# jonregef/sihl

Measured on NVIDIA B200. Metric: det-head images/sec (assign+loss+NMS), higher is better.
Workload: dtype f32

## Files before the change

### sihl_b200/csrc/od_nms.cu

```cuda
#include "od_common.cuh"

namespace sihl {

constexpr int kNmsThreads = 1024;
constexpr int kSmemItems = 4096;
constexpr int kBigSegment = 512;
constexpr int kSmallItems = 256;
static_assert(4 * kSmallItems == kNmsThreads, "short-list path: four lanes per candidate");
constexpr size_t kSmemItemBytes = 47;
constexpr size_t kWsItemBytes = 48;

__device__ __forceinline__ unsigned f2ord_nms(float f)
{
    const unsigned u = __float_as_uint(f);
    return (u & 0x80000000u) ? ~u : (u | 0x80000000u);
}

struct NmsArrays {
    unsigned long long *key;
    float4 *box;
    unsigned *val;
    float *area;
    unsigned *slot;
    int *seg;
    unsigned char *dead;
};

__device__ __forceinline__ NmsArrays carve(unsigned char *base, int np)
{
    NmsArrays a;
    a.key = reinterpret_cast<unsigned long long *>(base);
    a.box = reinterpret_cast<float4 *>(base + (size_t)np * 8);
    a.val = reinterpret_cast<unsigned *>(base + (size_t)np * 24);
    a.area = reinterpret_cast<float *>(base + (size_t)np * 28);
    a.slot = reinterpret_cast<unsigned *>(base + (size_t)np * 32);
    a.seg = reinterpret_cast<int *>(base + (size_t)np * 36);
    a.dead = base + (size_t)np * 40;
    return a;
}

template <bool DESC>
__device__ __forceinline__ void bitonic_kv(unsigned long long *key, unsigned *val, int np)
{
    for (int k = 2; k <= np; k <<= 1)
        for (int j = k >> 1; j > 0; j >>= 1) {
            for (int i = threadIdx.x; i < np; i += blockDim.x) {
                const int ixj = i ^ j;
                if (ixj > i) {
                    const unsigned long long a = key[i], b = key[ixj];
                    const bool first = (i & k) == 0;
                    const bool swap = DESC ? (first ? (a < b) : (a > b)) : (first ? (a > b) : (a < b));
                    if (swap) {
                        key[i] = b; key[ixj] = a;
                        if (val) { const unsigned t = val[i]; val[i] = val[ixj]; val[ixj] = t; }
                    }
                }
            }
            __syncthreads();
        }
}

template <class Flag, class Emit>
__device__ __forceinline__ int block_ordered_compact(int n, int *s_warp , Flag flag, Emit emit)
{
    const int lane = threadIdx.x & 31, warp = threadIdx.x >> 5, nwarps = blockDim.x >> 5;
    int running = 0;
    for (int i0 = 0; i0 < n; i0 += blockDim.x) {
        const int i = i0 + threadIdx.x;
        const bool f = i < n && flag(i);
        const unsigned m = __ballot_sync(kFullMask, f);
        if (lane == 0) s_warp[warp] = __popc(m);
        __syncthreads();
        if (warp == 0) {
            const int x = lane < nwarps ? s_warp[lane] : 0;
            int incl = x;
#pragma unroll
            for (int o = 1; o < 32; o <<= 1) {
                const int y = __shfl_up_sync(kFullMask, incl, o);
                if (lane >= o) incl += y;
            }
            if (lane < nwarps) s_warp[lane] = incl - x;
            if (lane == 31) s_warp[32] = incl;
        }
        __syncthreads();
        if (f) emit(i, running + s_warp[warp] + __popc(m & ((1u << lane) - 1u)));
        running += s_warp[32];
        __syncthreads();
    }
    return running;
}

__device__ __forceinline__ bool iou_gt(float4 a, float area_a, float4 b, float area_b, float thr)
{
    const float w = fmaxf(0.f, fminf(a.z, b.z) - fmaxf(a.x, b.x));
    const float h = fmaxf(0.f, fminf(a.w, b.w) - fmaxf(a.y, b.y));
    const float inter = w * h;
    return inter / ((area_a + area_b) - inter) > thr;
}

__device__ __forceinline__ float4 shfl4(float4 v, int src)
{
    return make_float4(__shfl_sync(kFullMask, v.x, src), __shfl_sync(kFullMask, v.y, src), __shfl_sync(kFullMask, v.z, src),
                       __shfl_sync(kFullMask, v.w, src));
}

__device__ __forceinline__ unsigned chunk_greedy(float4 bi, float ai, bool dead, float thr, int lane)
{
    unsigned over = 0u;
#pragma unroll 4
    for (int l = 0; l < 31; ++l) {
        const float4 bl = shfl4(bi, l);
        const float al = __shfl_sync(kFullMask, ai, l);
        if (l < lane && iou_gt(bl, al, bi, ai, thr)) over |= 1u << l;
    }
    const unsigned alive = __ballot_sync(kFullMask, !dead);
    unsigned kept = 0u;
#pragma unroll 4
    for (int l = 0; l < 32; ++l) {
        const unsigned ol = __shfl_sync(kFullMask, over, l);
        if (((alive >> l) & 1u) && (ol & kept) == 0u) kept |= 1u << l;
    }
    return kept;
}

template <bool SMEM>
__device__ __forceinline__ void warp_segment_nms(const float4 *box, const float *area, unsigned char *dead_flag, int q0, int m,
                                                 float thr, int lane)
{
    if (SMEM) { __builtin_assume(__isShared(box)); __builtin_assume(__isShared(area)); __builtin_assume(__isShared(dead_flag)); }
    else { __builtin_assume(__isGlobal(box)); __builtin_assume(__isGlobal(area)); __builtin_assume(__isGlobal(dead_flag)); }
    for (int c0 = 0; c0 < m; c0 += 32) {
        __syncwarp();
        const int i = c0 + lane;
        const bool valid = i < m;
        const float4 bi = valid ? box[q0 + i] : make_float4(0.f, 0.f, 0.f, 0.f);
        const float ai = valid ? area[q0 + i] : 0.f;
        const bool dead = valid ? dead_flag[q0 + i] != 0 : true;
        const unsigned kept = chunk_greedy(bi, ai, dead, thr, lane);
        if (valid && !dead && !((kept >> lane) & 1u)) dead_flag[q0 + i] = 1;
        for (int j0 = c0 + 32; j0 < m; j0 += 32) {
            const int j = j0 + lane;
            const bool live = j < m && dead_flag[q0 + j] == 0;
            const float4 bj = live ? box[q0 + j] : make_float4(0.f, 0.f, 0.f, 0.f);
            const float aj = live ? area[q0 + j] : 0.f;
            bool kill = false;
            for (unsigned k = kept; k != 0u; k &= k - 1u) {
                const int l = __ffs(k) - 1;
                const float4 bl = shfl4(bi, l);
                const float al = __shfl_sync(kFullMask, ai, l);
                if (live && !kill && iou_gt(bl, al, bj, aj, thr)) kill = true;
            }
            if (kill) dead_flag[q0 + j] = 1;
        }
    }
}

struct ChunkScratch { float4 box[32]; float area[32]; unsigned kept; int n_big; int big[32]; };

template <bool SMEM>
__device__ __forceinline__ void cta_segment_nms(const float4 *box, const float *area, unsigned char *dead_flag, int q0, int m,
                                                float thr, ChunkScratch *sc)
{
    if (SMEM) { __builtin_assume(__isShared(box)); __builtin_assume(__isShared(area)); __builtin_assume(__isShared(dead_flag)); }
    else { __builtin_assume(__isGlobal(box)); __builtin_assume(__isGlobal(area)); __builtin_assume(__isGlobal(dead_flag)); }
    __builtin_assume(__isShared(sc));
    const int tid = threadIdx.x, lane = tid & 31, warp = tid >> 5;
    for (int c0 = 0; c0 < m; c0 += 32) {
        __syncthreads();
        if (warp == 0) {
            const int i = c0 + lane;
            const bool valid = i < m;
            const float4 bi = valid ? box[q0 + i] : make_float4(0.f, 0.f, 0.f, 0.f);
            const float ai = valid ? area[q0 + i] : 0.f;
            const bool dead = valid ? dead_flag[q0 + i] != 0 : true;
            const unsigned kept = chunk_greedy(bi, ai, dead, thr, lane);
            if (valid && !dead && !((kept >> lane) & 1u)) dead_flag[q0 + i] = 1;
            sc->box[lane] = bi;
            sc->area[lane] = ai;
            if (lane == 0) sc->kept = kept;
        }
        __syncthreads();
        const unsigned kept = sc->kept;
        if (kept == 0u) continue;
        for (int j = c0 + 32 + tid; j < m; j += blockDim.x) {
            if (dead_flag[q0 + j]) continue;
            const float4 bj = box[q0 + j];
            const float aj = area[q0 + j];
            for (unsigned k = kept; k != 0u; k &= k - 1u) {
                const int l = __ffs(k) - 1;
                if (iou_gt(sc->box[l], sc->area[l], bj, aj, thr)) { dead_flag[q0 + j] = 1; break; }
            }
        }
    }
    __syncthreads();
}

struct NmsParams {
    const int32_t *cand_count; int64_t cap;
    const unsigned long long *cand_key; const float4 *cand_box; const int32_t *cand_cls;
    const float4 *boxes; const float *scores; const int64_t *classes; const int32_t *seg_offsets;
    int mode;
    float iou_thr;
    int K; int64_t *num_instances; float *out_scores; int64_t *out_classes; float4 *out_boxes;
    int64_t *keep; int32_t *keep_count;
    unsigned char *workspace; size_t ws_stride;
    int reset_counts;
    const int32_t *list_offsets;
    unsigned long long *out_keys;
    int smem_items;
};

__device__ __forceinline__ int64_t list_base(const NmsParams &p, int img)
{
    return p.list_offsets != nullptr ? (int64_t)__ldg(p.list_offsets + img) : (int64_t)img * p.cap;
}
__device__ __forceinline__ unsigned char *list_workspace(const NmsParams &p, int img, int src0)
{
    if (p.mode != 0) return p.workspace + (size_t)2 * src0 * kWsItemBytes;
    if (p.list_offsets != nullptr) return p.workspace + (size_t)2 * __ldg(p.list_offsets + img) * kWsItemBytes;
    return p.workspace + (size_t)img * p.ws_stride;
}

__device__ __forceinline__ void nms_big_body(const NmsParams &p)
{
    extern __shared__ __align__(16) unsigned char s_dyn[];
    __shared__ int s_warp[33];

    const int img = blockIdx.x, tid = threadIdx.x, lane = tid & 31, warp = tid >> 5, nwarps = blockDim.x >> 5;
    const int64_t lb = p.mode == 0 ? list_base(p, img) : 0;
    int n, src0;
    if (p.mode == 0) {
        const int c = __ldg(p.cand_count + img);
        n = (int)(c < p.cap ? c : p.cap);
        src0 = 0;
    } else {
        src0 = __ldg(p.seg_offsets + img);
        n = __ldg(p.seg_offsets + img + 1) - src0;
    }
    int np = 2;
    while (np < n) np <<= 1;
    int n_kept = 0;

    if (n > 0) {
        unsigned char *base = s_dyn;
        if (np > p.smem_items)
            base = list_workspace(p, img, src0);
        const NmsArrays ar = carve(base, np);

        for (int i = tid; i < np; i += blockDim.x) {
            unsigned long long key = 0ull;
            if (i < n) {
                if (p.mode == 0) key = __ldg(p.cand_key + lb + i);
                else key = ((unsigned long long)f2ord_nms(__ldg(p.scores + src0 + i)) << 32) |
                           (unsigned long long)(0xffffffffu - (unsigned)i);
            }
            ar.key[i] = key;
            ar.val[i] = (unsigned)i;
        }
        __syncthreads();
        bitonic_kv<true>(ar.key, ar.val, np);

        for (int r = tid; r < np; r += blockDim.x) {
            unsigned long long key = ~0ull;
            if (r < n) {
                const unsigned slot = ar.val[r];
                const unsigned c = p.mode == 0 ? (unsigned)__ldg(p.cand_cls + lb + slot)
                                               : (unsigned)__ldg(p.classes + src0 + slot);
                key = ((unsigned long long)c << 32) | (unsigned long long)r;
            }
            ar.key[r] = key;
        }
        __syncthreads();
        bitonic_kv<false>(ar.key, nullptr, np);
        for (int q = tid; q < n; q += blockDim.x) {
            const unsigned r = (unsigned)(ar.key[q] & 0xffffffffu), slot = ar.val[r];
            const float4 bx = p.mode == 0 ? __ldg(p.cand_box + lb + slot) : __ldg(p.boxes + src0 + slot);
            ar.box[q] = bx;
            ar.area[q] = (bx.z - bx.x) * (bx.w - bx.y);
            ar.slot[q] = slot;
            ar.dead[q] = 0;
        }
        __syncthreads();
        for (int q = tid; q < n; q += blockDim.x) ar.val[(unsigned)(ar.key[q] & 0xffffffffu)] = (unsigned)q;

        const int n_seg = block_ordered_compact(
            n, s_warp, [&](int q) { return q == 0 || (ar.key[q] >> 32) != (ar.key[q - 1] >> 32); },
            [&](int q, int s) { ar.seg[s] = q; });
        if (tid == 0) ar.seg[n_seg] = n;
        __syncthreads();
        bool any_big = false;
        for (int s = warp; s < n_seg; s += nwarps) {
            const int q0 = ar.seg[s], m = ar.seg[s + 1] - q0;
            if (m > kBigSegment) continue;
            for (int i = 0; i + 1 < m; ++i) {
                __syncwarp();
                if (ar.dead[q0 + i]) continue;
                const float4 bi = ar.box[q0 + i];
                const float ai = ar.area[q0 + i];
                for (int j = i + 1 + lane; j < m; j += 32)
                    if (!ar.dead[q0 + j] && iou_gt(bi, ai, ar.box[q0 + j], ar.area[q0 + j], p.iou_thr)) ar.dead[q0 + j] = 1;
            }
        }
        for (int s = 0; s < n_seg; ++s) any_big |= (ar.seg[s + 1] - ar.seg[s]) > kBigSegment;
        __syncthreads();
        if (any_big) {
            for (int s = 0; s < n_seg; ++s) {
                const int q0 = ar.seg[s], m = ar.seg[s + 1] - q0;
                if (m <= kBigSegment) continue;
                for (int i = 0; i + 1 < m; ++i) {
                    __syncthreads();
                    if (ar.dead[q0 + i]) continue;
                    const float4 bi = ar.box[q0 + i];
                    const float ai = ar.area[q0 + i];
                    for (int j = i + 1 + tid; j < m; j += blockDim.x)
                        if (!ar.dead[q0 + j] && iou_gt(bi, ai, ar.box[q0 + j], ar.area[q0 + j], p.iou_thr))
                            ar.dead[q0 + j] = 1;
                }
                __syncthreads();
            }
        }

        n_kept = block_ordered_compact(
            n, s_warp, [&](int r) { return ar.dead[ar.val[r]] == 0; },
            [&](int r, int k) {
                const unsigned q = ar.val[r], slot = ar.slot[q];
                if (p.mode == 0) {
                    if (k < p.K) {
                        const int64_t o = (int64_t)img * p.K + k;
                        const unsigned long long ck = __ldg(p.cand_key + lb + slot);
                        p.out_scores[o] = __uint_as_float((unsigned)(ck >> 32));
                        p.out_classes[o] = (int64_t)(ar.key[q] >> 32);
                        p.out_boxes[o] = ar.box[q];
                        if (p.out_keys != nullptr) p.out_keys[o] = ck;
                    }
                } else {
                    p.keep[src0 + k] = (int64_t)src0 + slot;
                }
            });
    }

    if (p.mode == 0) {
        const int m = n_kept < p.K ? n_kept : p.K;
        if (tid == 0) {
            p.num_instances[img] = m;
            if (p.reset_counts) const_cast<int32_t *>(p.cand_count)[img] = 0;
        }
        for (int k = m + tid; k < p.K; k += blockDim.x) {
            const int64_t o = (int64_t)img * p.K + k;
            p.out_scores[o] = 0.f;
            p.out_classes[o] = 0;
            p.out_boxes[o] = make_float4(0.f, 0.f, 0.f, 0.f);
        }
    } else if (tid == 0) {
        p.keep_count[img] = n_kept;
    }
}

__device__ __forceinline__ int nms_small_body(const NmsParams &p, const int *sel = nullptr, int n_sel = 0, bool finalize = true)
{
    __shared__ unsigned long long s_key[kSmallItems];
    __shared__ unsigned s_cls[kSmallItems];
    __shared__ float4 s_box[kSmallItems];
    __shared__ float s_area[kSmallItems];
    __shared__ unsigned s_mask[kSmallItems];
    __shared__ unsigned s_keep[kSmallItems];
    __shared__ unsigned char s_dead[kSmallItems];
    __shared__ unsigned short s_q_of_r[kSmallItems], s_slot_of_r[kSmallItems], s_seg0_of_q[kSmallItems], s_len_of_q[kSmallItems];
    __shared__ int s_warp[33];
    __shared__ int s_big;

    const int img = blockIdx.x, tid = threadIdx.x, lane = tid & 31;
    const int64_t lb = p.mode == 0 ? list_base(p, img) : 0;
    const int item = tid >> 2, sub = tid & 3;
    int n, src0;
    if (p.mode == 0) {
        const int c = __ldg(p.cand_count + img);
        n = (int)(c < p.cap ? c : p.cap);
        src0 = 0;
    } else {
        src0 = __ldg(p.seg_offsets + img);
        n = __ldg(p.seg_offsets + img + 1) - src0;
    }
    if (sel != nullptr) n = n_sel;
    int n_kept = 0;
    if (n > 0) {
        const bool have = item < n;
        unsigned long long key = 0ull;
        unsigned cls = 0;
        float4 bx = make_float4(0.f, 0.f, 0.f, 0.f);
        if (have) {
            if (p.mode == 0) {
                const int src = sel != nullptr ? sel[item] : item;
                key = __ldg(p.cand_key + lb + src);
                cls = (unsigned)__ldg(p.cand_cls + lb + src);
                bx = __ldg(p.cand_box + lb + src);
            } else {
                key = ((unsigned long long)f2ord_nms(__ldg(p.scores + src0 + item)) << 32) |
                      (unsigned long long)(0xffffffffu - (unsigned)item);
                cls = (unsigned)__ldg(p.classes + src0 + item);
                bx = __ldg(p.boxes + src0 + item);
            }
            if (sub == 0) { s_key[item] = key; s_cls[item] = cls; }
        }
        if (tid == 0) s_big = 0;
        if (sub == 0 && item < kSmallItems) {
            s_q_of_r[item] = 0; s_slot_of_r[item] = 0; s_seg0_of_q[item] = 0; s_len_of_q[item] = 1; s_mask[item] = 0u;
            s_keep[item] = 0u; s_dead[item] = 0; s_box[item] = make_float4(0.f, 0.f, 0.f, 0.f); s_area[item] = 0.f;
        }
        __syncthreads();
        int r = 0, seg0 = 0, k = 0, len = 0;
        if (have) {
#pragma unroll 4
            for (int j = sub; j < n; j += 4) {
                const unsigned long long kj = s_key[j];
                const unsigned cj = s_cls[j];
                const bool better = kj > key, same = cj == cls;
                r += better;
                seg0 += cj < cls;
                k += same && better;
                len += same;
            }
        }
#pragma unroll
        for (int o = 2; o > 0; o >>= 1) {
            r += __shfl_xor_sync(kFullMask, r, o);
            seg0 += __shfl_xor_sync(kFullMask, seg0, o);
            k += __shfl_xor_sync(kFullMask, k, o);
            len += __shfl_xor_sync(kFullMask, len, o);
        }
        const int q = seg0 + k;
        if (have && sub == 0) {
            s_box[q] = bx;
            s_area[q] = (bx.z - bx.x) * (bx.w - bx.y);
            s_q_of_r[r] = (unsigned short)q;
            s_slot_of_r[r] = (unsigned short)item;
            s_seg0_of_q[q] = (unsigned short)seg0;
            s_len_of_q[q] = (unsigned short)len;
            s_dead[q] = 0;
            if (len > 32) s_big = 1;
        }
        __syncthreads();
        unsigned mask = 0;
        if (have && len <= 32) {
            const float area = (bx.z - bx.x) * (bx.w - bx.y);
            for (int j = sub; j < k; j += 4)
                if (iou_gt(s_box[seg0 + j], s_area[seg0 + j], bx, area, p.iou_thr)) mask |= 1u << j;
        }
        mask |= __shfl_xor_sync(kFullMask, mask, 1);
        mask |= __shfl_xor_sync(kFullMask, mask, 2);
        if (have && sub == 0) s_mask[q] = mask;
        __syncthreads();
        if (have && sub == 0 && k == 0 && len <= 32) {
            unsigned kept = 1u;
            for (int i = 1; i < len; ++i)
                if ((s_mask[seg0 + i] & kept) == 0u) kept |= 1u << i;
            s_keep[seg0] = kept;
        }
        __syncthreads();
        if (s_big) {
            const int warp = tid >> 5, nwarps = blockDim.x >> 5;
            for (int qq = warp; qq < n; qq += nwarps) {
                const int q0 = s_seg0_of_q[qq], m = s_len_of_q[qq];
                if (qq != q0 || m <= 32) continue;
                for (int i = 0; i + 1 < m; ++i) {
                    __syncwarp();
                    if (s_dead[q0 + i]) continue;
                    const float4 bi = s_box[q0 + i];
                    const float ai = s_area[q0 + i];
                    for (int j = i + 1 + lane; j < m; j += 32)
                        if (!s_dead[q0 + j] && iou_gt(bi, ai, s_box[q0 + j], s_area[q0 + j], p.iou_thr)) s_dead[q0 + j] = 1;
                }
            }
            __syncthreads();
        }
        n_kept = block_ordered_compact(
            n, s_warp,
            [&](int rr) {
                const int qq = s_q_of_r[rr], q0 = s_seg0_of_q[qq];
                return s_len_of_q[qq] <= 32 ? ((s_keep[q0] >> (qq - q0)) & 1u) != 0u : s_dead[qq] == 0;
            },
            [&](int rr, int kk) {
                const int qq = s_q_of_r[rr], slot = s_slot_of_r[rr];
                if (p.mode == 0) {
                    if (kk < p.K) {
                        const int64_t o = (int64_t)img * p.K + kk;
                        p.out_scores[o] = __uint_as_float((unsigned)(s_key[slot] >> 32));
                        p.out_classes[o] = (int64_t)s_cls[slot];
                        p.out_boxes[o] = s_box[qq];
                        if (p.out_keys != nullptr) p.out_keys[o] = s_key[slot];
                    }
                } else {
                    p.keep[src0 + kk] = (int64_t)src0 + slot;
                }
            });
    }
    if (!finalize) return n_kept;
    if (p.mode == 0) {
        const int m = n_kept < p.K ? n_kept : p.K;
        if (tid == 0) {
            p.num_instances[img] = m;
            if (p.reset_counts) const_cast<int32_t *>(p.cand_count)[img] = 0;
        }
        for (int kk = m + tid; kk < p.K; kk += blockDim.x) {
            const int64_t o = (int64_t)img * p.K + kk;
            p.out_scores[o] = 0.f;
            p.out_classes[o] = 0;
            p.out_boxes[o] = make_float4(0.f, 0.f, 0.f, 0.f);
        }
    } else if (tid == 0) {
        p.keep_count[img] = n_kept;
    }
    return n_kept;
}

constexpr int kLazyTarget = 200;
constexpr int kLazyMaxK = 128;
__device__ __forceinline__ int lazy_prefix_select(const NmsParams &p, int64_t lb, int n, int *s_sel, unsigned *s_hist,
                                                  unsigned *s_pick, int *s_count)
{
    const int tid = threadIdx.x, lane = tid & 31;
    unsigned prefix = 0u, mask = 0u, remaining = (unsigned)kLazyTarget;
    for (int pass = 0; pass < 4; ++pass) {
        const int shift = 24 - 8 * pass;
        for (int i = tid; i < 256; i += blockDim.x) s_hist[i] = 0u;
        __syncthreads();
        for (int i0 = 0; i0 < n; i0 += blockDim.x) {
            const int i = i0 + tid;
            const bool ok = i < n;
            const unsigned u = ok ? (unsigned)(__ldg(p.cand_key + lb + i) >> 32) : 0u;
            const bool in = ok && ((u & mask) == prefix);
            const unsigned digit = (u >> shift) & 255u;
            const unsigned act = __ballot_sync(kFullMask, in);
            if (in) {
                const unsigned peers = __match_any_sync(act, digit);
                if (lane == __ffs(peers) - 1) atomicAdd(&s_hist[digit], (unsigned)__popc(peers));
            }
        }
        __syncthreads();
        if (tid < 32) {
            unsigned c[8], tot = 0u;
#pragma unroll
            for (int j = 0; j < 8; ++j) { c[j] = s_hist[255 - (lane * 8 + j)]; tot += c[j]; }
            unsigned incl = tot;
#pragma unroll
            for (int o = 1; o < 32; o <<= 1) {
                const unsigned y = __shfl_up_sync(kFullMask, incl, o);
                if (lane >= o) incl += y;
            }
            unsigned before = incl - tot;
            if (before < remaining && remaining <= incl) {
#pragma unroll
                for (int j = 0; j < 8; ++j) {
                    if (before < remaining && remaining <= before + c[j]) {
                        s_pick[0] = 255u - (unsigned)(lane * 8 + j);
                        s_pick[1] = remaining - before;
                    }
                    before += c[j];
                }
            }
        }
        __syncthreads();
        prefix |= s_pick[0] << shift;
        mask |= 255u << shift;
        remaining = s_pick[1];
        __syncthreads();
    }
    if (tid == 0) *s_count = 0;
    __syncthreads();
    for (int i0 = 0; i0 < n; i0 += blockDim.x) {
        const int i = i0 + tid;
        if (i < n && (unsigned)(__ldg(p.cand_key + lb + i) >> 32) >= prefix) {
            const int pos = atomicAdd(s_count, 1);
            if (pos < kSmallItems) s_sel[pos] = i;
        }
    }
    __syncthreads();
    const int c = *s_count;
    return c <= kSmallItems ? c : 0;
}

constexpr int kWarpSegment = 2048;
constexpr int kHashSlots = 1024;
constexpr unsigned kHashEmpty = 0xffffffffu;
constexpr size_t kMedItemBytes = 47;
static_assert(kMedItemBytes <= kSmemItemBytes && kMedItemBytes <= kWsItemBytes, "long-list layouts must fit the shared/workspace strides");

struct MedArrays {
    unsigned long long *u_key;
    unsigned long long *f_key;
    float4 *f_box;
    unsigned *u_slot, *f_slot;
    float *f_area;
    unsigned short *b_id;
    unsigned char *f_dead;
};

__device__ __forceinline__ MedArrays carve_med(unsigned char *base, int n_al)
{
    MedArrays a;
    a.u_key = reinterpret_cast<unsigned long long *>(base);
    a.f_key = reinterpret_cast<unsigned long long *>(base + (size_t)n_al * 8);
    a.f_box = reinterpret_cast<float4 *>(base + (size_t)n_al * 16);
    a.u_slot = reinterpret_cast<unsigned *>(base + (size_t)n_al * 32);
    a.f_slot = reinterpret_cast<unsigned *>(base + (size_t)n_al * 36);
    a.f_area = reinterpret_cast<float *>(base + (size_t)n_al * 40);
    a.b_id = reinterpret_cast<unsigned short *>(base + (size_t)n_al * 44);
    a.f_dead = base + (size_t)n_al * 46;
    return a;
}

template <bool SMEM>
__device__ __forceinline__ bool nms_medium_body(const NmsParams &p, int n, int src0, unsigned char *base, int n_al,
                                                int *s_warp, unsigned *h_cls, int *h_cnt, int *h_start, ChunkScratch *chunk_scratch,
                                                int *n_kept_out)
{
    if (SMEM) __builtin_assume(__isShared(base));
    else __builtin_assume(__isGlobal(base));
    __builtin_assume(__isShared(h_cls));
    __builtin_assume(__isShared(h_cnt));
    __builtin_assume(__isShared(h_start));
    int &s_distinct = h_start[0];
    const int img = blockIdx.x, tid = threadIdx.x, lane = tid & 31, warp = tid >> 5, nwarps = blockDim.x >> 5;
    const int64_t lb = p.mode == 0 ? list_base(p, img) : 0;
    const MedArrays ar = carve_med(base, n_al);

    auto key_of = [&](int i) -> unsigned long long {
        if (p.mode == 0) return __ldg(p.cand_key + lb + i);
        return ((unsigned long long)f2ord_nms(__ldg(p.scores + src0 + i)) << 32) | (unsigned long long)(0xffffffffu - (unsigned)i);
    };
    auto cls_of = [&](int i) -> unsigned {
        return p.mode == 0 ? (unsigned)__ldg(p.cand_cls + lb + i) : (unsigned)__ldg(p.classes + src0 + i);
    };

    for (int h = tid; h < kHashSlots; h += blockDim.x) { h_cls[h] = kHashEmpty; h_cnt[h] = 0; }
    if (tid == 0) s_distinct = 0;
    __syncthreads();
    for (int i = tid; i < n; i += blockDim.x) {
        const unsigned c = cls_of(i);
        unsigned h = (c * 2654435761u) >> 22;
        for (int probe = 0; probe < kHashSlots; ++probe) {
            const unsigned prev = atomicCAS(&h_cls[h], kHashEmpty, c);
            if (prev == kHashEmpty) { atomicAdd(&s_distinct, 1); break; }
            if (prev == c) break;
            h = (h + 1) & (kHashSlots - 1);
        }
        ar.b_id[i] = (unsigned short)h;
        atomicAdd(&h_cnt[h], 1);
    }
    __syncthreads();
    if (s_distinct > kHashSlots / 2) return false;
    {
        const int c = tid < kHashSlots ? h_cnt[tid] : 0;
        int incl = c;
#pragma unroll
        for (int o = 1; o < 32; o <<= 1) {
            const int y = __shfl_up_sync(kFullMask, incl, o);
            if (lane >= o) incl += y;
        }
        if (lane == 31) s_warp[warp] = incl;
        __syncthreads();
        if (warp == 0) {
            const int x = lane < nwarps ? s_warp[lane] : 0;
            int wi = x;
#pragma unroll
            for (int o = 1; o < 32; o <<= 1) {
                const int y = __shfl_up_sync(kFullMask, wi, o);
                if (lane >= o) wi += y;
            }
            s_warp[lane] = wi - x;
        }
        __syncthreads();
        if (tid < kHashSlots) { h_start[tid] = s_warp[warp] + incl - c; h_cnt[tid] = 0; }
    }
    __syncthreads();
    for (int i = tid; i < n; i += blockDim.x) {
        const int h = ar.b_id[i];
        const int pos = h_start[h] + atomicAdd(&h_cnt[h], 1);
        ar.u_key[pos] = key_of(i);
        ar.u_slot[pos] = (unsigned)i;
    }
    __syncthreads();
    for (int pp = tid; pp < n; pp += blockDim.x) {
        const unsigned long long key = ar.u_key[pp];
        const unsigned slot = ar.u_slot[pp];
        const int h = ar.b_id[slot];
        const int s0 = h_start[h], e0 = s0 + h_cnt[h];
        int rank = 0;
        if (p.mode == 0) {
            for (int j = s0; j < e0; ++j) {
                const unsigned long long kj = ar.u_key[j];
                rank += kj > key || (kj == key && j < pp);
            }
        } else {
            for (int j = s0; j < e0; ++j) rank += ar.u_key[j] > key;
        }
        const int q = s0 + rank;
        const float4 bx = p.mode == 0 ? __ldg(p.cand_box + lb + slot) : __ldg(p.boxes + src0 + slot);
        ar.f_key[q] = key;
        ar.f_slot[q] = slot;
        ar.f_box[q] = bx;
        ar.f_area[q] = (bx.z - bx.x) * (bx.w - bx.y);
        ar.f_dead[q] = 0;
    }
    __syncthreads();
    unsigned long long *mask = ar.u_key;
    if (tid == 0) chunk_scratch->n_big = 0;
    for (int q = tid; q < n; q += blockDim.x) {
        const int h = ar.b_id[ar.f_slot[q]];
        const int s0 = h_start[h], m = h_cnt[h];
        unsigned long long bits = 0ull;
        if (m <= 64) {
            const float4 bq = ar.f_box[q];
            const float aq = ar.f_area[q];
            for (int j = s0; j < q; ++j)
                if (iou_gt(ar.f_box[j], ar.f_area[j], bq, aq, p.iou_thr)) bits |= 1ull << (j - s0);
        }
        mask[q] = bits;
    }
    __syncthreads();
    for (int h = tid; h < kHashSlots; h += blockDim.x) {
        const int m = h_cnt[h];
        if (m > kWarpSegment) {
            const int k = atomicAdd(&chunk_scratch->n_big, 1);
            if (k < 32) chunk_scratch->big[k] = h;
        }
        if (m < 2 || m > 64) continue;
        const int s0 = h_start[h];
        unsigned long long kept = 1ull;
        for (int i = 1; i < m; ++i) {
            if ((mask[s0 + i] & kept) == 0ull) kept |= 1ull << i;
            else ar.f_dead[s0 + i] = 1;
        }
    }
    for (int h = warp; h < kHashSlots; h += nwarps) {
        const int m = h_cnt[h];
        if (m <= 64 || m > kWarpSegment) continue;
        warp_segment_nms<SMEM>(ar.f_box, ar.f_area, ar.f_dead, h_start[h], m, p.iou_thr, lane);
    }
    __syncthreads();
    const int n_big = chunk_scratch->n_big;
    if (n_big > 0) {
        if (n_big <= 32) {
            for (int k = 0; k < n_big; ++k) {
                const int h = chunk_scratch->big[k];
                cta_segment_nms<SMEM>(ar.f_box, ar.f_area, ar.f_dead, h_start[h], h_cnt[h], p.iou_thr, chunk_scratch);
            }
        } else {
            for (int h = 0; h < kHashSlots; ++h)
                if (h_cnt[h] > kWarpSegment)
                    cta_segment_nms<SMEM>(ar.f_box, ar.f_area, ar.f_dead, h_start[h], h_cnt[h], p.iou_thr, chunk_scratch);
        }
    }
    const int n_kept = block_ordered_compact(
        n, s_warp, [&](int q) { return ar.f_dead[q] == 0; },
        [&](int q, int k) { ar.u_key[k] = ar.f_key[q]; ar.u_slot[k] = (unsigned)q; });
    __syncthreads();
    auto emit = [&](int k_src, int rank) {
        const unsigned q = ar.u_slot[k_src], slot = ar.f_slot[q];
        if (p.mode == 0) {
            const int64_t o = (int64_t)img * p.K + rank;
            p.out_scores[o] = __uint_as_float((unsigned)(ar.u_key[k_src] >> 32));
            p.out_classes[o] = (int64_t)h_cls[ar.b_id[slot]];
            p.out_boxes[o] = ar.f_box[q];
            if (p.out_keys != nullptr) p.out_keys[o] = ar.u_key[k_src];
        } else {
            p.keep[src0 + rank] = (int64_t)src0 + slot;
        }
    };
    const int want = p.mode == 0 ? (n_kept < p.K ? n_kept : p.K) : n_kept;
    if (p.mode == 1 && n_kept > 4096) {
        int np = 2;
        while (np < n_kept) np <<= 1;
        for (int k = n_kept + tid; k < np; k += blockDim.x) { ar.u_key[k] = 0ull; ar.u_slot[k] = 0u; }
        __syncthreads();
        bitonic_kv<true>(ar.u_key, ar.u_slot, np);
        for (int k = tid; k < n_kept; k += blockDim.x) emit(k, k);
    } else {
        unsigned thr_hi = 0u;
        if (n_kept > want) {
            unsigned *hist = reinterpret_cast<unsigned *>(h_cnt);
            unsigned prefix = 0, mask = 0, remaining = (unsigned)want;
            for (int pass = 0; pass < 4; ++pass) {
                const int shift = 24 - 8 * pass;
                for (int i = tid; i < 256; i += blockDim.x) hist[i] = 0;
                __syncthreads();
                for (int k0 = 0; k0 < n_kept; k0 += blockDim.x) {
                    const int k = k0 + tid;
                    const bool ok = k < n_kept;
                    const unsigned u = ok ? (unsigned)(ar.u_key[k] >> 32) : 0u;
                    const bool in = ok && ((u & mask) == prefix);
                    const unsigned digit = (u >> shift) & 255u;
                    const unsigned act = __ballot_sync(kFullMask, in);
                    if (in) {
                        const unsigned peers = __match_any_sync(act, digit);
                        if (lane == __ffs(peers) - 1) atomicAdd(&hist[digit], (unsigned)__popc(peers));
                    }
                }
                __syncthreads();
                if (warp == 0) {
                    unsigned c[8], tot = 0;
#pragma unroll
                    for (int j = 0; j < 8; ++j) { c[j] = hist[255 - (lane * 8 + j)]; tot += c[j]; }
                    unsigned incl = tot;
#pragma unroll
                    for (int o = 1; o < 32; o <<= 1) {
                        const unsigned y = __shfl_up_sync(kFullMask, incl, o);
                        if (lane >= o) incl += y;
                    }
                    unsigned before = incl - tot;
                    if (before < remaining && remaining <= incl) {
#pragma unroll
                        for (int j = 0; j < 8; ++j) {
                            if (before < remaining && remaining <= before + c[j]) {
                                hist[256] = 255u - (unsigned)(lane * 8 + j);
                                hist[257] = remaining - before;
                            }
                            before += c[j];
                        }
                    }
                }
                __syncthreads();
                prefix |= hist[256] << shift;
                mask |= 255u << shift;
                remaining = hist[257];
                __syncthreads();
            }
            thr_hi = prefix;
        }
        unsigned long long *pass_key = ar.f_key;
        unsigned *pass_src = reinterpret_cast<unsigned *>(ar.f_area);
        __syncthreads();
        const int n_pass = block_ordered_compact(
            n_kept, s_warp, [&](int k) { return (unsigned)(ar.u_key[k] >> 32) >= thr_hi; },
            [&](int k, int r) { pass_key[r] = ar.u_key[k]; pass_src[r] = (unsigned)k; });
        __syncthreads();
        for (int r = tid; r < n_pass; r += blockDim.x) {
            const unsigned long long key = pass_key[r];
            int rank = 0;
            if (p.mode == 0) {
                for (int j = 0; j < n_pass; ++j) rank += pass_key[j] > key || (pass_key[j] == key && j < r);
            } else {
                for (int j = 0; j < n_pass; ++j) rank += pass_key[j] > key;
            }
            if (rank < want) emit((int)pass_src[r], rank);
        }
    }
    *n_kept_out = n_kept;
    return true;
}

__global__ void __launch_bounds__(kNmsThreads) k_nms(NmsParams p)
{
    extern __shared__ __align__(16) unsigned char s_dyn_top[];
    __shared__ int s_warp_top[33];
    __shared__ unsigned s_hcls[kHashSlots];
    __shared__ int s_hcnt[kHashSlots], s_hstart[kHashSlots];
    __shared__ ChunkScratch s_chunk;
    int n, src0;
    if (p.mode == 0) {
        const int c = __ldg(p.cand_count + blockIdx.x);
        n = (int)(c < p.cap ? c : p.cap);
        src0 = 0;
    } else {
        src0 = __ldg(p.seg_offsets + blockIdx.x);
        n = __ldg(p.seg_offsets + blockIdx.x + 1) - src0;
    }
    if (n <= kSmallItems) { nms_small_body(p); return; }
    if (p.mode == 0 && p.K <= kLazyMaxK) {
        __shared__ int s_sel[kSmallItems];
        __shared__ unsigned s_pick[2];
        __shared__ int s_count;
        const int64_t lb = list_base(p, (int)blockIdx.x);
        const int m = lazy_prefix_select(p, lb, n, s_sel, reinterpret_cast<unsigned *>(s_hcnt), s_pick, &s_count);
        if (m > 0) {
            const int kept = nms_small_body(p, s_sel, m, false);
            if (kept >= p.K) {
                if (threadIdx.x == 0) {
                    p.num_instances[blockIdx.x] = p.K;
                    if (p.reset_counts) const_cast<int32_t *>(p.cand_count)[blockIdx.x] = 0;
                }
                return;
            }
            __syncthreads();
        }
    }
    int n_al = 2;
    while (n_al < n) n_al <<= 1;
    int n_kept = 0;
    bool done;
    if (n_al <= p.smem_items) {
        done = nms_medium_body<true>(p, n, src0, s_dyn_top, n_al, s_warp_top, s_hcls, s_hcnt, s_hstart, &s_chunk, &n_kept);
    } else {
        unsigned char *ws = list_workspace(p, (int)blockIdx.x, src0);
        done = nms_medium_body<false>(p, n, src0, ws, n_al, s_warp_top, s_hcls, s_hcnt, s_hstart, &s_chunk, &n_kept);
    }
    if (done) {
        const int img = blockIdx.x, tid = threadIdx.x;
        if (p.mode == 0) {
            const int m = n_kept < p.K ? n_kept : p.K;
            if (tid == 0) {
                p.num_instances[img] = m;
                if (p.reset_counts) const_cast<int32_t *>(p.cand_count)[img] = 0;
            }
            for (int k = m + tid; k < p.K; k += blockDim.x) {
                const int64_t o = (int64_t)img * p.K + k;
                p.out_scores[o] = 0.f;
                p.out_classes[o] = 0;
                p.out_boxes[o] = make_float4(0.f, 0.f, 0.f, 0.f);
            }
        } else if (tid == 0) {
            p.keep_count[img] = n_kept;
        }
        return;
    }
    __syncthreads();
    nms_big_body(p);
}

constexpr int kMaxSplit = 64;

__device__ __forceinline__ int sub_list_of(unsigned cls, int S) { return (int)(((cls * 2654435761u) >> 16) % (unsigned)S); }

struct SplitParams {
    int32_t *cand_count; int64_t cap;
    const unsigned long long *key; const float4 *box; const int32_t *cls;
    int S; int32_t *sub_count; int32_t *sub_offset;
    unsigned long long *key2; float4 *box2; int32_t *cls2;
    int reset_counts;
};

__global__ void __launch_bounds__(1024) k_nms_split_lists(SplitParams p)
{
    __shared__ int s_cnt[kMaxSplit], s_start[kMaxSplit], s_cur[kMaxSplit];
    const int img = blockIdx.x, tid = threadIdx.x, S = p.S;
    const int c = __ldg(p.cand_count + img);
    const int n = (int)(c < p.cap ? c : p.cap);
    const int64_t lb = (int64_t)img * p.cap;
    if (tid < kMaxSplit) { s_cnt[tid] = 0; s_cur[tid] = 0; }
    __syncthreads();
    for (int i = tid; i < n; i += blockDim.x) atomicAdd(&s_cnt[sub_list_of((unsigned)__ldg(p.cls + lb + i), S)], 1);
    __syncthreads();
    if (tid == 0) {
        int run = 0;
        for (int s = 0; s < S; ++s) { s_start[s] = run; run += s_cnt[s]; }
    }
    __syncthreads();
    for (int i = tid; i < n; i += blockDim.x) {
        const int cl = __ldg(p.cls + lb + i);
        const int s = sub_list_of((unsigned)cl, S);
        const int64_t dst = lb + s_start[s] + atomicAdd(&s_cur[s], 1);
        p.key2[dst] = __ldg(p.key + lb + i);
        p.box2[dst] = __ldg(p.box + lb + i);
        p.cls2[dst] = cl;
    }
    if (tid < S) {
        p.sub_count[img * S + tid] = s_cnt[tid];
        p.sub_offset[img * S + tid] = (int32_t)(lb + s_start[tid]);
    }
    if (tid == 0 && p.reset_counts) p.cand_count[img] = 0;
}

struct MergeParams {
    int S, K;
    const int64_t *sub_num; const unsigned long long *sub_keys; const float *sub_scores; const int64_t *sub_classes;
    const float4 *sub_boxes;
    int64_t *num_instances; float *out_scores; int64_t *out_classes; float4 *out_boxes;
};

template <bool STAGED>
__global__ void __launch_bounds__(512) k_nms_merge(MergeParams p)
{
    extern __shared__ __align__(16) unsigned char s_merge[];
    __shared__ int s_num[kMaxSplit];
    const int img = blockIdx.x, tid = threadIdx.x, S = p.S, K = p.K;
    if (tid < S) s_num[tid] = (int)__ldg(p.sub_num + img * S + tid);
    __syncthreads();
    const unsigned long long *keys = p.sub_keys + (int64_t)img * S * K;
    if (STAGED) {
        unsigned long long *sk = reinterpret_cast<unsigned long long *>(s_merge);
        for (int e = tid; e < S * K; e += blockDim.x) {
            const int s = e / K, k = e - s * K;
            if (k < s_num[s]) sk[e] = __ldg(keys + e);
        }
        __syncthreads();
        keys = sk;
    }
    int total = 0;
    for (int s = 0; s < S; ++s) total += s_num[s];
    const int m = total < K ? total : K;
    for (int e = tid; e < S * K; e += blockDim.x) {
        const int s = e / K, k = e - s * K;
        if (k >= s_num[s]) continue;
        const unsigned long long key = keys[e];
        int rank = k;
        for (int t = 0; t < S && rank < K; ++t) {
            if (t == s) continue;
            const unsigned long long *other = keys + t * K;
            int lo = 0, hi = s_num[t];
            while (lo < hi) {
                const int mid = (lo + hi) >> 1;
                if (other[mid] > key) lo = mid + 1; else hi = mid;
            }
            rank += lo;
        }
        if (rank < K) {
            const int64_t src = ((int64_t)img * S + s) * K + k;
            const int64_t o = (int64_t)img * K + rank;
            p.out_scores[o] = __ldg(p.sub_scores + src);
            p.out_classes[o] = __ldg(p.sub_classes + src);
            p.out_boxes[o] = __ldg(p.sub_boxes + src);
        }
    }
    if (tid == 0) p.num_instances[img] = m;
    for (int k = m + tid; k < K; k += blockDim.x) {
        const int64_t o = (int64_t)img * K + k;
        p.out_scores[o] = 0.f;
        p.out_classes[o] = 0;
        p.out_boxes[o] = make_float4(0.f, 0.f, 0.f, 0.f);
    }
}

static int pow2ceil(int64_t n)
{
    int p = 2;
    while (p < n) p <<= 1;
    return p;
}

static int launch_nms(NmsParams p, int n_images, int64_t max_items, cudaStream_t st, int smem_items = kSmemItems)
{
    p.smem_items = smem_items;
    const size_t smem = max_items > kSmallItems ? (size_t)smem_items * kSmemItemBytes : 0;
    static thread_local bool attr_set = false;
    if (smem && !attr_set) {
        int rc = cuda_status(cudaFuncSetAttribute(k_nms, cudaFuncAttributeMaxDynamicSharedMemorySize,
                                                  (int)((size_t)kSmemItems * kSmemItemBytes)),
                             "cudaFuncSetAttribute(k_nms)");
        if (rc) return rc;
        attr_set = true;
    }
    k_nms<<<n_images, kNmsThreads, smem, st>>>(p);
    SIHL_CHECK_LAUNCH("k_nms");
    return SIHL_OD_OK;
}

}

using namespace sihl;

extern "C" size_t sihl_od_nms_workspace_bytes(int batch, int64_t cand_capacity)
{
    if (batch <= 0 || cand_capacity <= 0) return 0;
    const int np = pow2ceil(cand_capacity);
    if (np <= kSmemItems) return 0;
    return (size_t)batch * (size_t)np * kWsItemBytes;
}

extern "C" int sihl_od_nms_topk(const int32_t *cand_count, int64_t cand_capacity, const uint64_t *cand_key,
                                const float *cand_box, const int32_t *cand_cls, int batch, float iou_thr, int k,
                                int64_t *num_instances, float *scores, int64_t *classes, float *boxes, void *workspace,
                                int reset_counts, void *stream)
{
    SIHL_CHECK_ARG(cand_count && cand_key && cand_box && cand_cls, "NULL input");
    SIHL_CHECK_ARG(num_instances && scores && classes && boxes, "NULL output");
    SIHL_CHECK_ARG(cand_capacity >= 1 && cand_capacity < (1ll << 30) && k >= 1, "bad sizes");
    SIHL_CHECK_ARG(workspace != nullptr || sihl_od_nms_workspace_bytes(batch, cand_capacity) == 0,
                   "workspace needed for capacity %lld", (long long)cand_capacity);
    if (batch <= 0) return SIHL_OD_OK;
    NmsParams p = {};
    p.cand_count = cand_count; p.cap = cand_capacity;
    p.cand_key = reinterpret_cast<const unsigned long long *>(cand_key);
    p.cand_box = reinterpret_cast<const float4 *>(cand_box); p.cand_cls = cand_cls;
    p.mode = 0; p.iou_thr = iou_thr; p.K = k; p.reset_counts = reset_counts;
    p.num_instances = num_instances; p.out_scores = scores; p.out_classes = classes;
    p.out_boxes = reinterpret_cast<float4 *>(boxes);
    p.workspace = static_cast<unsigned char *>(workspace);
    p.ws_stride = (size_t)pow2ceil(cand_capacity) * kWsItemBytes;
    return launch_nms(p, batch, cand_capacity, (cudaStream_t)stream);
}

namespace sihl {
size_t wide_nms_workspace_bytes(int64_t n);
bool wide_nms_applies(int64_t n);
int launch_wide_batched_nms(const float *boxes, const float *scores, const int64_t *classes, const int32_t *seg_offsets,
                            int n_images, int64_t n, float iou_thr, int64_t *keep, int32_t *keep_count, void *workspace,
                            cudaStream_t st);
}

extern "C" size_t sihl_od_batched_nms_workspace_bytes(int64_t n)
{
    if (wide_nms_applies(n)) return wide_nms_workspace_bytes(n);
    if (n <= kSmemItems) return 0;
    return (size_t)(2 * n + 2) * kWsItemBytes;
}

extern "C" int sihl_od_batched_nms(const float *boxes, const float *scores, const int64_t *classes,
                                   const int32_t *seg_offsets, int n_images, int64_t n, float iou_thr, int64_t *keep,
                                   int32_t *keep_count, void *workspace, void *stream)
{
    SIHL_CHECK_ARG(seg_offsets && keep_count, "NULL argument");
    SIHL_CHECK_ARG(n >= 0 && n < (1ll << 30) && n_images >= 0, "bad sizes");
    SIHL_CHECK_ARG(n == 0 || (boxes && scores && classes && keep), "NULL argument");
    SIHL_CHECK_ARG(workspace != nullptr || sihl_od_batched_nms_workspace_bytes(n) == 0, "workspace needed for n=%lld",
                   (long long)n);
    if (n_images == 0) return SIHL_OD_OK;
    if (wide_nms_applies(n))
        return launch_wide_batched_nms(boxes, scores, classes, seg_offsets, n_images, n, iou_thr, keep, keep_count, workspace,
                                       (cudaStream_t)stream);
    NmsParams p = {};
    p.boxes = reinterpret_cast<const float4 *>(boxes); p.scores = scores; p.classes = classes; p.seg_offsets = seg_offsets;
    p.mode = 1; p.iou_thr = iou_thr; p.keep = keep; p.keep_count = keep_count;
    p.workspace = static_cast<unsigned char *>(workspace); p.ws_stride = 0;
    return launch_nms(p, n_images, n, (cudaStream_t)stream);
}

static int split_factor(int64_t cand_capacity)
{
    int64_t s = (cand_capacity + 2047) / 2048;
    if (s < 2) s = 2;
    if (s > 32) s = 32;
    return (int)s;
}

static size_t align256(size_t x) { return (x + 255) / 256 * 256; }

extern "C" size_t sihl_od_nms_split_workspace_bytes(int batch, int64_t cand_capacity, int k)
{
    if (batch <= 0 || cand_capacity <= 0 || k <= 0) return 0;
    const size_t S = (size_t)split_factor(cand_capacity), B = (size_t)batch, cap = (size_t)cand_capacity, K = (size_t)k;
    size_t bytes = 0;
    bytes += align256(B * cap * 8) + align256(B * cap * 16) + align256(B * cap * 4);
    bytes += 2 * align256(B * S * 4);
    bytes += align256(B * S * 8) + align256(B * S * K * 8) + align256(B * S * K * 4) + align256(B * S * K * 8) +
             align256(B * S * K * 16);
    bytes += align256((size_t)(2 * B * cap + 2) * kWsItemBytes);
    return bytes;
}

extern "C" int sihl_od_nms_topk_split(int32_t *cand_count, int64_t cand_capacity, const uint64_t *cand_key,
                                      const float *cand_box, const int32_t *cand_cls, int batch, float iou_thr, int k,
                                      int64_t *num_instances, float *scores, int64_t *classes, float *boxes, void *workspace,
                                      int reset_counts, void *stream)
{
    SIHL_CHECK_ARG(cand_count && cand_key && cand_box && cand_cls, "NULL input");
    SIHL_CHECK_ARG(num_instances && scores && classes && boxes && workspace, "NULL output / workspace");
    SIHL_CHECK_ARG(cand_capacity >= 1 && (int64_t)batch * cand_capacity < (1ll << 30) && k >= 1 && k <= 4096, "bad sizes");
    if (batch <= 0) return SIHL_OD_OK;
    cudaStream_t st = (cudaStream_t)stream;
    const int S = split_factor(cand_capacity);
    const size_t B = (size_t)batch, cap = (size_t)cand_capacity, K = (size_t)k;
    unsigned char *w = static_cast<unsigned char *>(workspace);
    auto take = [&](size_t bytes) { unsigned char *ptr = w; w += align256(bytes); return ptr; };
    SplitParams sp;
    sp.cand_count = cand_count; sp.cap = cand_capacity;
    sp.key = reinterpret_cast<const unsigned long long *>(cand_key); sp.box = reinterpret_cast<const float4 *>(cand_box);
    sp.cls = cand_cls; sp.S = S; sp.reset_counts = reset_counts;
    sp.key2 = reinterpret_cast<unsigned long long *>(take(B * cap * 8));
    sp.box2 = reinterpret_cast<float4 *>(take(B * cap * 16));
    sp.cls2 = reinterpret_cast<int32_t *>(take(B * cap * 4));
    sp.sub_count = reinterpret_cast<int32_t *>(take(B * S * 4));
    sp.sub_offset = reinterpret_cast<int32_t *>(take(B * S * 4));
    int64_t *sub_num = reinterpret_cast<int64_t *>(take(B * S * 8));
    unsigned long long *sub_keys = reinterpret_cast<unsigned long long *>(take(B * S * K * 8));
    float *sub_scores = reinterpret_cast<float *>(take(B * S * K * 4));
    int64_t *sub_classes = reinterpret_cast<int64_t *>(take(B * S * K * 8));
    float4 *sub_boxes = reinterpret_cast<float4 *>(take(B * S * K * 16));
    unsigned char *nms_ws = take((size_t)(2 * B * cap + 2) * kWsItemBytes);
    k_nms_split_lists<<<batch, 1024, 0, st>>>(sp);
    SIHL_CHECK_LAUNCH("k_nms_split_lists");
    NmsParams p = {};
    p.cand_count = sp.sub_count; p.cap = cand_capacity; p.list_offsets = sp.sub_offset;
    p.cand_key = sp.key2; p.cand_box = sp.box2; p.cand_cls = sp.cls2;
    p.mode = 0; p.iou_thr = iou_thr; p.K = k; p.reset_counts = 0;
    p.num_instances = sub_num; p.out_scores = sub_scores; p.out_classes = sub_classes; p.out_boxes = sub_boxes;
    p.out_keys = sub_keys; p.workspace = nms_ws; p.ws_stride = 0;
    int rc = launch_nms(p, batch * S, cand_capacity, st, kSmemItems / 2);
    if (rc) return rc;
    MergeParams mp;
    mp.S = S; mp.K = k; mp.sub_num = sub_num; mp.sub_keys = sub_keys; mp.sub_scores = sub_scores; mp.sub_classes = sub_classes;
    mp.sub_boxes = sub_boxes; mp.num_instances = num_instances; mp.out_scores = scores; mp.out_classes = classes;
    mp.out_boxes = reinterpret_cast<float4 *>(boxes);
    const size_t stage = (size_t)S * K * 8;
    if (stage <= 96 * 1024) {
        static thread_local bool merge_attr = false;
        if (!merge_attr) {
            rc = cuda_status(cudaFuncSetAttribute(k_nms_merge<true>, cudaFuncAttributeMaxDynamicSharedMemorySize, 96 * 1024),
                             "cudaFuncSetAttribute(k_nms_merge)");
            if (rc) return rc;
            merge_attr = true;
        }
        k_nms_merge<true><<<batch, 512, stage, st>>>(mp);
    } else {
        k_nms_merge<false><<<batch, 512, 0, st>>>(mp);
    }
    SIHL_CHECK_LAUNCH("k_nms_merge");
    return SIHL_OD_OK;
}
```

Before: 1.590 million.

## Run top-k NMS with 512-thread blocks and global-memory workspace instead of shared

Templates the NMS kernel on block size and launches the top-k detection path with 512 threads (two lanes per candidate in the short-list path, two hash slots per thread in the scan) and two blocks per SM. That path now passes zero dynamic shared memory, so medium lists use the global workspace, and the workspace size rule changes to match. The aim is more resident blocks and less shared-memory pressure per image, at the cost of global-memory traffic for lists longer than 256 and less parallelism per candidate.

```diff
diff --git a/sihl_b200/csrc/od_nms.cu b/sihl_b200/csrc/od_nms.cu
--- a/sihl_b200/csrc/od_nms.cu
+++ b/sihl_b200/csrc/od_nms.cu
@@ -2,11 +2,11 @@
 
 namespace sihl {
 
-constexpr int kNmsThreads = 1024;
+constexpr int kNmsThreadsTopk = 512;
+constexpr int kNmsThreadsAlone = 1024;
 constexpr int kSmemItems = 4096;
 constexpr int kBigSegment = 512;
 constexpr int kSmallItems = 256;
-static_assert(4 * kSmallItems == kNmsThreads, "short-list path: four lanes per candidate");
 constexpr size_t kSmemItemBytes = 47;
 constexpr size_t kWsItemBytes = 48;
 
@@ -356,8 +356,11 @@
     }
 }
 
+template <int THREADS>
 __device__ __forceinline__ int nms_small_body(const NmsParams &p, const int *sel = nullptr, int n_sel = 0, bool finalize = true)
 {
+    constexpr int kLanes = THREADS / kSmallItems;
+    static_assert(kLanes * kSmallItems == THREADS && (kLanes == 2 || kLanes == 4), "short-list path: 2 or 4 lanes per candidate");
     __shared__ unsigned long long s_key[kSmallItems];
     __shared__ unsigned s_cls[kSmallItems];
     __shared__ float4 s_box[kSmallItems];
@@ -371,7 +374,7 @@
 
     const int img = blockIdx.x, tid = threadIdx.x, lane = tid & 31;
     const int64_t lb = p.mode == 0 ? list_base(p, img) : 0;
-    const int item = tid >> 2, sub = tid & 3;
+    const int item = tid / kLanes, sub = tid % kLanes;
     int n, src0;
     if (p.mode == 0) {
         const int c = __ldg(p.cand_count + img);
@@ -411,7 +414,7 @@
         int r = 0, seg0 = 0, k = 0, len = 0;
         if (have) {
 #pragma unroll 4
-            for (int j = sub; j < n; j += 4) {
+            for (int j = sub; j < n; j += kLanes) {
                 const unsigned long long kj = s_key[j];
                 const unsigned cj = s_cls[j];
                 const bool better = kj > key, same = cj == cls;
@@ -422,7 +425,7 @@
             }
         }
 #pragma unroll
-        for (int o = 2; o > 0; o >>= 1) {
+        for (int o = kLanes / 2; o > 0; o >>= 1) {
             r += __shfl_xor_sync(kFullMask, r, o);
             seg0 += __shfl_xor_sync(kFullMask, seg0, o);
             k += __shfl_xor_sync(kFullMask, k, o);
@@ -443,11 +446,11 @@
         unsigned mask = 0;
         if (have && len <= 32) {
             const float area = (bx.z - bx.x) * (bx.w - bx.y);
-            for (int j = sub; j < k; j += 4)
+            for (int j = sub; j < k; j += kLanes)
                 if (iou_gt(s_box[seg0 + j], s_area[seg0 + j], bx, area, p.iou_thr)) mask |= 1u << j;
         }
-        mask |= __shfl_xor_sync(kFullMask, mask, 1);
-        mask |= __shfl_xor_sync(kFullMask, mask, 2);
+#pragma unroll
+        for (int o = kLanes / 2; o > 0; o >>= 1) mask |= __shfl_xor_sync(kFullMask, mask, o);
         if (have && sub == 0) s_mask[q] = mask;
         __syncthreads();
         if (have && sub == 0 && k == 0 && len <= 32) {
@@ -609,7 +612,7 @@
     return a;
 }
 
-template <bool SMEM>
+template <bool SMEM, int THREADS>
 __device__ __forceinline__ bool nms_medium_body(const NmsParams &p, int n, int src0, unsigned char *base, int n_al,
                                                 int *s_warp, unsigned *h_cls, int *h_cnt, int *h_start, ChunkScratch *chunk_scratch,
                                                 int *n_kept_out)
@@ -650,7 +653,11 @@
     __syncthreads();
     if (s_distinct > kHashSlots / 2) return false;
     {
-        const int c = tid < kHashSlots ? h_cnt[tid] : 0;
+        constexpr int kSlotsPerThread = kHashSlots / THREADS;
+        static_assert(kSlotsPerThread * THREADS == kHashSlots, "hash slots split evenly over the threads");
+        int cs[kSlotsPerThread], c = 0;
+#pragma unroll
+        for (int j = 0; j < kSlotsPerThread; ++j) { cs[j] = h_cnt[kSlotsPerThread * tid + j]; c += cs[j]; }
         int incl = c;
 #pragma unroll
         for (int o = 1; o < 32; o <<= 1) {
@@ -670,7 +677,13 @@
             s_warp[lane] = wi - x;
         }
         __syncthreads();
-        if (tid < kHashSlots) { h_start[tid] = s_warp[warp] + incl - c; h_cnt[tid] = 0; }
+        int run = s_warp[warp] + incl - c;
+#pragma unroll
+        for (int j = 0; j < kSlotsPerThread; ++j) {
+            h_start[kSlotsPerThread * tid + j] = run;
+            h_cnt[kSlotsPerThread * tid + j] = 0;
+            run += cs[j];
+        }
     }
     __syncthreads();
     for (int i = tid; i < n; i += blockDim.x) {
@@ -849,7 +862,8 @@
     return true;
 }
 
-__global__ void __launch_bounds__(kNmsThreads) k_nms(NmsParams p)
+template <int THREADS>
+__global__ void __launch_bounds__(THREADS, 1024 / THREADS) k_nms(NmsParams p)
 {
     extern __shared__ __align__(16) unsigned char s_dyn_top[];
     __shared__ int s_warp_top[33];
@@ -865,7 +879,7 @@
         src0 = __ldg(p.seg_offsets + blockIdx.x);
         n = __ldg(p.seg_offsets + blockIdx.x + 1) - src0;
     }
-    if (n <= kSmallItems) { nms_small_body(p); return; }
+    if (n <= kSmallItems) { nms_small_body<THREADS>(p); return; }
     if (p.mode == 0 && p.K <= kLazyMaxK) {
         __shared__ int s_sel[kSmallItems];
         __shared__ unsigned s_pick[2];
@@ -873,7 +887,7 @@
         const int64_t lb = list_base(p, (int)blockIdx.x);
         const int m = lazy_prefix_select(p, lb, n, s_sel, reinterpret_cast<unsigned *>(s_hcnt), s_pick, &s_count);
         if (m > 0) {
-            const int kept = nms_small_body(p, s_sel, m, false);
+            const int kept = nms_small_body<THREADS>(p, s_sel, m, false);
             if (kept >= p.K) {
                 if (threadIdx.x == 0) {
                     p.num_instances[blockIdx.x] = p.K;
@@ -889,10 +903,10 @@
     int n_kept = 0;
     bool done;
     if (n_al <= p.smem_items) {
-        done = nms_medium_body<true>(p, n, src0, s_dyn_top, n_al, s_warp_top, s_hcls, s_hcnt, s_hstart, &s_chunk, &n_kept);
+        done = nms_medium_body<true, THREADS>(p, n, src0, s_dyn_top, n_al, s_warp_top, s_hcls, s_hcnt, s_hstart, &s_chunk, &n_kept);
     } else {
         unsigned char *ws = list_workspace(p, (int)blockIdx.x, src0);
-        done = nms_medium_body<false>(p, n, src0, ws, n_al, s_warp_top, s_hcls, s_hcnt, s_hstart, &s_chunk, &n_kept);
+        done = nms_medium_body<false, THREADS>(p, n, src0, ws, n_al, s_warp_top, s_hcls, s_hcnt, s_hstart, &s_chunk, &n_kept);
     }
     if (done) {
         const int img = blockIdx.x, tid = threadIdx.x;
@@ -1027,19 +1041,20 @@
     return p;
 }
 
-static int launch_nms(NmsParams p, int n_images, int64_t max_items, cudaStream_t st, int smem_items = kSmemItems)
+template <int THREADS>
+static int launch_nms(NmsParams p, int n_images, int64_t max_items, cudaStream_t st, int smem_items)
 {
     p.smem_items = smem_items;
     const size_t smem = max_items > kSmallItems ? (size_t)smem_items * kSmemItemBytes : 0;
     static thread_local bool attr_set = false;
     if (smem && !attr_set) {
-        int rc = cuda_status(cudaFuncSetAttribute(k_nms, cudaFuncAttributeMaxDynamicSharedMemorySize,
+        int rc = cuda_status(cudaFuncSetAttribute(k_nms<THREADS>, cudaFuncAttributeMaxDynamicSharedMemorySize,
                                                   (int)((size_t)kSmemItems * kSmemItemBytes)),
                              "cudaFuncSetAttribute(k_nms)");
         if (rc) return rc;
         attr_set = true;
     }
-    k_nms<<<n_images, kNmsThreads, smem, st>>>(p);
+    k_nms<THREADS><<<n_images, THREADS, smem, st>>>(p);
     SIHL_CHECK_LAUNCH("k_nms");
     return SIHL_OD_OK;
 }
@@ -1052,7 +1067,7 @@
 {
     if (batch <= 0 || cand_capacity <= 0) return 0;
     const int np = pow2ceil(cand_capacity);
-    if (np <= kSmemItems) return 0;
+    if (np <= kSmallItems) return 0;
     return (size_t)batch * (size_t)np * kWsItemBytes;
 }
 
@@ -1076,7 +1091,7 @@
     p.out_boxes = reinterpret_cast<float4 *>(boxes);
     p.workspace = static_cast<unsigned char *>(workspace);
     p.ws_stride = (size_t)pow2ceil(cand_capacity) * kWsItemBytes;
-    return launch_nms(p, batch, cand_capacity, (cudaStream_t)stream);
+    return launch_nms<kNmsThreadsTopk>(p, batch, cand_capacity, (cudaStream_t)stream, 0);
 }
 
 namespace sihl {
@@ -1111,7 +1126,7 @@
     p.boxes = reinterpret_cast<const float4 *>(boxes); p.scores = scores; p.classes = classes; p.seg_offsets = seg_offsets;
     p.mode = 1; p.iou_thr = iou_thr; p.keep = keep; p.keep_count = keep_count;
     p.workspace = static_cast<unsigned char *>(workspace); p.ws_stride = 0;
-    return launch_nms(p, n_images, n, (cudaStream_t)stream);
+    return launch_nms<kNmsThreadsAlone>(p, n_images, n, (cudaStream_t)stream, kSmemItems);
 }
 
 static int split_factor(int64_t cand_capacity)
@@ -1174,7 +1189,7 @@
     p.mode = 0; p.iou_thr = iou_thr; p.K = k; p.reset_counts = 0;
     p.num_instances = sub_num; p.out_scores = sub_scores; p.out_classes = sub_classes; p.out_boxes = sub_boxes;
     p.out_keys = sub_keys; p.workspace = nms_ws; p.ws_stride = 0;
-    int rc = launch_nms(p, batch * S, cand_capacity, st, kSmemItems / 2);
+    int rc = launch_nms<kNmsThreadsAlone>(p, batch * S, cand_capacity, st, kSmemItems / 2);
     if (rc) return rc;
     MergeParams mp;
     mp.S = S; mp.K = k; mp.sub_num = sub_num; mp.sub_keys = sub_keys; mp.sub_scores = sub_scores; mp.sub_classes = sub_classes;
```

Result: faster. 1.734 million, median of 6 (+9.1%).
